# 0xPARC/plonkathon

Measured on NVIDIA H100. Metric: plonk_proofs_per_s_2^20_gates, higher is better.
Workload: dtype u256 (BN254 Fr/Fq integers, 8x32-bit Montgomery limbs)

## Files before the change

plonkathon_b200/csrc/capi.cu:

```cuda
#include "../../include/plonk_b200.h"

#include <cstring>

#include "common.cuh"
#include "comm.cuh"
#include "msm_bucket.cuh"
#include "prover.cuh"
#include "pairing.cuh"
#include "transcript.cuh"

namespace pb200 {
void ntt_run(Context* ctx, const Fr* in, Fr* out, int log_n, bool inverse, uint64_t n_in, const Fr* in_scale,
             const Fr* out_scale);
void launch_powers(Context* ctx, Fr* out, uint64_t n, const Fr& base, const Fr& scale);
Fr fr_from_u64(uint64_t x);
void ntt_run_strided(Context* ctx, const Fr* in, Fr* out, int log_n, bool inverse, uint64_t n_in,
                     const Fr* in_scale, const Fr* out_scale, uint64_t in_mul, uint64_t in_add);
void ntt_sharded(Context* ctx, const Fr* const* in, Fr* const* out, int count, int log_n, bool inverse);
void fr_to_mont(Context* ctx, const Fr* in, Fr* out, uint64_t n);
void fr_from_mont(Context* ctx, const Fr* in, Fr* out, uint64_t n);
void fr_vec_op(Context* ctx, int op, const Fr* a, const Fr* b, const Fr& scalar_canonical, Fr* out, uint64_t n,
               uint64_t shift);
void barycentric_eval(Context* ctx, const Fr* d_vals, int log_n, const Fr& x_mont, Fr* h_out);
float bench_modmul(Context* ctx, int field, uint64_t threads, uint32_t iters);
struct Srs;
Srs* srs_create(Context* ctx, const uint8_t* h_points, uint64_t n, int precompute);
void srs_destroy(Srs* s);
Srs* srs_generate(Context* ctx, const Fr& tau_canonical, uint64_t n, int precompute);
Srs* srs_generate_lagrange(Context* ctx, const Fr& tau_canonical, uint64_t n, int precompute);
void srs_export(Context* ctx, Srs* srs, uint8_t* h_points, uint64_t first, uint64_t count);
void srs_msm(Context* ctx, Srs* srs, const Fr* d_scalars, uint64_t m, bool scalars_mont, uint8_t* out_xy, int* is_identity);
uint64_t srs_size(Srs* s);
uint32_t msm_default_window(uint64_t n, bool fixed_base);
void msm_run(Context* ctx, const G1Affine* points, uint64_t n, const Fr* scalars, bool scalars_mont, uint32_t c,
             bool fixed_base, uint64_t point_stride, uint8_t* out_xy, int* is_identity);
void affine_to_mont(Context* ctx, const G1Affine* in, G1Affine* out, uint64_t n);
Prover* prover_create(Context* ctx, Srs* srs, int log_n, const uint8_t* const* h_pk, int n_custom,
                      const uint8_t* h_exps, const uint8_t* const* h_custom, bool sharded, int exp_width);
void prover_destroy(Prover* p);
void prover_prove(Prover* P, const uint8_t* hA, const uint8_t* hB, const uint8_t* hC, const uint8_t* h_public,
                  uint64_t n_public, uint8_t* out, bool wires_on_device);
void prover_round1(Prover* P, const uint8_t* hA, const uint8_t* hB, const uint8_t* hC, const uint8_t* h_public,
                   uint64_t n_public, bool wires_on_device);
void prover_round2(Prover* P, const Fr* ch);
void prover_round3(Prover* P, const Fr& alpha_c, const Fr& cofactor_c);
void prover_round4(Prover* P, const Fr& zeta_c);
void prover_round5(Prover* P, const Fr& v_c);
void prover_serialize(const Prover* P, uint8_t* out);
size_t copy_step(const Prover* P, int step, uint8_t* out);
void prover_set_zk(Prover* P, unsigned block, bool enable, const uint8_t* h_blinders);
void prover_set_lookup(Prover* P, const uint8_t* h_qk, const uint8_t* h_qtag, const uint8_t* const* h_tab,
                       uint64_t rows);
void prover_round_lookup(Prover* P, const Fr& eta_c);
void prover_set_shuffle(Prover* P, const uint8_t* h_qin, const uint8_t* h_qout);
void g1_combine_partials_host(const G1XYZZ* parts, uint32_t count, uint8_t* out_xy, int* is_identity);
void host_join_bucket_shards(const SR* all, uint32_t world, uint32_t sets, uint32_t nloc, G1XYZZ* out);
void host_join_bucket_shards_strided(const SR* all, uint32_t world, uint32_t sets, G1XYZZ* out);
void prover_check(Prover* P, const uint8_t* hA, const uint8_t* hB, const uint8_t* hC, const uint8_t* h_public,
                  uint64_t n_public, uint32_t limit, uint64_t* h_counts, uint32_t* h_lists, bool wires_on_device);
void permutation_run(Context* ctx, const int64_t* h_ids, int log_n, uint8_t* h_S);
Srs* srs_create_ptau(Context* ctx, const uint8_t* h_g1, uint64_t count, const uint8_t* h_tau_g2, int precompute);
Srs* srs_create_ptau_lagrange(Context* ctx, const uint8_t* h_block, uint64_t n, Srs* monomial, int precompute);
void ptau_stages(double* out_ms, int count);

const Bn254Pairing& pairing_engine() {
  static const Bn254Pairing engine;
  return engine;
}
}

using namespace pb200;

static thread_local std::string g_err;

#define PB_API_BEGIN try {
#define PB_API_END                        \
  return 0;                               \
  }                                       \
  catch (const std::exception& e) {       \
    g_err = e.what();                     \
    return 1;                             \
  }                                       \
  catch (...) {                           \
    g_err = "unknown error";              \
    return 1;                             \
  }
// ... 67 lines not shown
                  const uint8_t* y, uint8_t* out) {
  PB_API_BEGIN PB_ON_CTX(reinterpret_cast<Prover*>(p)->ctx);
  Prover* P = reinterpret_cast<Prover*>(p);
  require_kind(P, kind, "round2", STEP_2);
  Fr ch[PROOF_CHALLENGES] = {};
  ch[CH_BETA] = load_fr_canonical(beta);
  ch[CH_GAMMA] = load_fr_canonical(gamma);
  if (kind != BLOCK_PLAIN) {
    const bool sh = kind & BLOCK_SHUFFLE;
    ch[sh ? CH_THETA : CH_DELTA] = load_fr_canonical(x);
    ch[sh ? CH_KAPPA : CH_EPSILON] = load_fr_canonical(y);
  }
  prover_round2(P, ch);
  copy_step(P, STEP_2, out);
  PB_API_END
}
static int round4(pb200_prover* p, unsigned kind, const uint8_t* zeta, uint8_t* out) {
  PB_API_BEGIN PB_ON_CTX(reinterpret_cast<Prover*>(p)->ctx);
  Prover* P = reinterpret_cast<Prover*>(p);
  require_kind(P, kind, "round4", STEP_4);
  prover_round4(P, load_fr_canonical(zeta));
  copy_step(P, STEP_4, out);
  PB_API_END
}
static int set_zk(pb200_prover* p, unsigned block, int enable, const uint8_t* h_blinders) {
  PB_API_BEGIN PB_ON_CTX(reinterpret_cast<Prover*>(p)->ctx);
  prover_set_zk(reinterpret_cast<Prover*>(p), block, enable != 0, h_blinders);
  PB_API_END
}

extern "C" {

const char* pb200_last_error(void) { return g_err.c_str(); }
const char* pb200_version(void) { return "plonk_b200 0.1 (sm_90a)"; }

int pb200_ctx_create(int device, void* cuda_stream, pb200_ctx** out) {
  PB_API_BEGIN
  int count = 0;
  cudaError_t e = cudaGetDeviceCount(&count);
  PB_CHECK(e == cudaSuccess && count > 0, "no CUDA device: libplonk_b200 has no CPU fallback");
  PB_CHECK(device >= 0 && device < count, "bad device ordinal");
  PB_CUDA(cudaSetDevice(device));
  auto ctx = std::make_unique<Context>();
  ctx->device = device;
  cudaDeviceProp prop;
  PB_CUDA(cudaGetDeviceProperties(&prop, device));
  ctx->sm_count = prop.multiProcessorCount;
  if (cuda_stream) {
    ctx->stream = reinterpret_cast<cudaStream_t>(cuda_stream);
  } else {
    PB_CUDA(cudaStreamCreateWithFlags(&ctx->stream, cudaStreamNonBlocking));
    ctx->own_stream = true;
  }
  *out = reinterpret_cast<pb200_ctx*>(ctx.release());
  PB_API_END
}

void pb200_ctx_destroy(pb200_ctx* ctx) {
  if (!ctx) return;
  cudaSetDevice(C(ctx)->device);
  cudaStreamSynchronize(C(ctx)->stream);
  delete C(ctx);
}

int pb200_ctx_sync(pb200_ctx* ctx) {
  PB_API_BEGIN PB_ON_CTX(C(ctx));
  PB_CUDA(cudaStreamSynchronize(C(ctx)->stream));
  PB_API_END
}

uint64_t pb200_ctx_launches(pb200_ctx* ctx) { return C(ctx)->launches; }

int pb200_ctx_timing(pb200_ctx* ctx, int enable) {
  PB_API_BEGIN PB_ON_CTX(C(ctx));
  Context* c = C(ctx);
  PB_CUDA(cudaStreamSynchronize(c->stream));
  for (auto& v : c->timed) {
    for (auto& pr : v) { cudaEventDestroy(pr.first); cudaEventDestroy(pr.second); }
    v.clear();
  }
  c->timing = enable != 0;
  PB_API_END
}
int pb200_ctx_timing_read(pb200_ctx* ctx, int category, double* total_ms, uint64_t* count) {
  PB_API_BEGIN PB_ON_CTX(C(ctx));
  Context* c = C(ctx);
  PB_CHECK(category >= 0 && category < 4, "bad timing category");
  PB_CUDA(cudaStreamSynchronize(c->stream));
  double t = 0;
  for (auto& pr : c->timed[category]) {
    float ms = 0;
    PB_CUDA(cudaEventElapsedTime(&ms, pr.first, pr.second));
    t += ms;
  }
  *total_ms = t;
  *count = c->timed[category].size();
  PB_API_END
}
void* pb200_ctx_stream(pb200_ctx* ctx) { return (void*)C(ctx)->stream; }

int pb200_fr_to_mont(pb200_ctx* ctx, const void* d_in, void* d_out, uint64_t n) {
  PB_API_BEGIN PB_ON_CTX(C(ctx));
  fr_to_mont(C(ctx), (const Fr*)d_in, (Fr*)d_out, n);
  PB_API_END
}
int pb200_fr_from_mont(pb200_ctx* ctx, const void* d_in, void* d_out, uint64_t n) {
// ... 582 lines not shown
```

plonkathon_b200/csrc/common.cuh:

```cuda
#pragma once
#include <cuda_runtime.h>
#include <stdint.h>
#include <stdio.h>
#include <map>
#include <memory>
#include <stdexcept>
#include <string>
#include <vector>

#include "curve.cuh"
#include "field.cuh"
#include "modinv.cuh"

namespace pb200 {

struct Error : std::runtime_error {
  using std::runtime_error::runtime_error;
};

#define PB_CUDA(expr)                                                                          \
  do {                                                                                         \
    cudaError_t e__ = (expr);                                                                  \
    if (e__ != cudaSuccess) {                                                                  \
      char b__[512];                                                                           \
      snprintf(b__, sizeof b__, "%s failed: %s (%s:%d)", #expr, cudaGetErrorString(e__),       \
               __FILE__, __LINE__);                                                            \
      throw pb200::Error(b__);                                                                 \
    }                                                                                          \
  } while (0)

#define PB_CHECK(cond, msg)                                                                    \
  do {                                                                                         \
    if (!(cond)) {                                                                             \
      char b__[512];                                                                           \
      snprintf(b__, sizeof b__, "%s (%s:%d)", msg, __FILE__, __LINE__);                        \
      throw pb200::Error(b__);                                                                 \
    }                                                                                          \
  } while (0)

struct DevBuf {
  void* p = nullptr;
  size_t bytes = 0;
  DevBuf() {}
  explicit DevBuf(size_t n) { alloc(n); }
  DevBuf(const DevBuf&) = delete;
  DevBuf& operator=(const DevBuf&) = delete;
  DevBuf(DevBuf&& o) noexcept : p(o.p), bytes(o.bytes) { o.p = nullptr; o.bytes = 0; }
  DevBuf& operator=(DevBuf&& o) noexcept {
    if (this != &o) { release(); p = o.p; bytes = o.bytes; o.p = nullptr; o.bytes = 0; }
    return *this;
  }
  ~DevBuf() { release(); }
  void alloc(size_t n) {
    release();
    if (n) PB_CUDA(cudaMalloc(&p, n));
    bytes = n;
  }
  void ensure(size_t n) { if (n > bytes) alloc(n); }
  void release() { if (p) cudaFree(p); p = nullptr; bytes = 0; }
  template <class T> T* as() const { return reinterpret_cast<T*>(p); }
};

struct NttPlan;
struct Srs;
struct Comm;
struct ShardTables;

struct Context {
  int device = 0;
  cudaStream_t stream = nullptr;
  bool own_stream = false;
  cudaStream_t aux_stream = nullptr;
  cudaEvent_t aux_ev[4] = {nullptr, nullptr, nullptr, nullptr};
  cudaStream_t copy_stream = nullptr;
  cudaEvent_t copy_done[4] = {nullptr, nullptr, nullptr, nullptr};
  int sm_count = 132;
  std::map<int, std::unique_ptr<NttPlan>> plans;
  DevBuf scratch[10];
  DevBuf msm_aff[6];
  Comm* comm = nullptr;
  DevBuf gather;
  std::map<int, std::unique_ptr<ShardTables>> shard_tables;
  uint64_t launches = 0;
  bool timing = false;
  std::vector<std::pair<cudaEvent_t, cudaEvent_t>> timed[4];
  void time_begin(int cat) {
    if (!timing) return;
    cudaEvent_t a, b;
    cudaEventCreate(&a);
    cudaEventCreate(&b);
    cudaEventRecord(a, stream);
    timed[cat].push_back({a, b});
  }
  void time_end(int cat) {
    if (!timing) return;
    cudaEventRecord(timed[cat].back().second, stream);
  }
  Context();
  ~Context();
};

NttPlan* get_plan(Context* ctx, int log_n, bool inverse);

}
```

plonkathon_b200/csrc/msm.cu:

```cuda
#include <algorithm>
#include <cstring>

#include "common.cuh"
#include "comm.cuh"
#include "msm_bucket.cuh"
#include "msm_digits.cuh"
#include "msm_sort.cuh"

namespace pb200 {

__device__ __forceinline__ G1Affine ld_affine(const G1Affine* p) {
  const uint4* q = reinterpret_cast<const uint4*>(p);
  uint4 a = __ldg(q), b = __ldg(q + 1), c = __ldg(q + 2), d = __ldg(q + 3);
  G1Affine r;
  r.x.v[0] = a.x; r.x.v[1] = a.y; r.x.v[2] = a.z; r.x.v[3] = a.w;
  r.x.v[4] = b.x; r.x.v[5] = b.y; r.x.v[6] = b.z; r.x.v[7] = b.w;
  r.y.v[0] = c.x; r.y.v[1] = c.y; r.y.v[2] = c.z; r.y.v[3] = c.w;
  r.y.v[4] = d.x; r.y.v[5] = d.y; r.y.v[6] = d.z; r.y.v[7] = d.w;
  return r;
}

__device__ __forceinline__ uint32_t block_exclusive_scan(uint32_t v, uint32_t* sh, uint32_t* total) {
  const uint32_t lane = threadIdx.x & 31, wid = threadIdx.x >> 5, nw = blockDim.x >> 5;
  uint32_t x = v;
  for (int d = 1; d < 32; d <<= 1) {
    uint32_t y = __shfl_up_sync(0xffffffffu, x, d);
    if ((int)lane >= d) x += y;
  }
  if (lane == 31) sh[wid] = x;
  __syncthreads();
  if (wid == 0) {
    uint32_t w = lane < nw ? sh[lane] : 0;
    for (int d = 1; d < 32; d <<= 1) {
      uint32_t y = __shfl_up_sync(0xffffffffu, w, d);
      if ((int)lane >= d) w += y;
    }
    if (lane < nw) sh[lane] = w;
  }
  __syncthreads();
  uint32_t base = wid ? sh[wid - 1] : 0;
  *total = sh[nw - 1];
  __syncthreads();
  return base + x - v;
}

__global__ void __launch_bounds__(PB_SORT_BIN_THREADS) k_msm_bin_count(SortArgs a) {
  __shared__ uint32_t sh_cnt[PB_SORT_MAX_BINS];
  const uint32_t t = threadIdx.x, nt = blockDim.x;
  sort_zero(sh_cnt, a.nbins, t, nt);
  __syncthreads();
  bin_hist(a, blockIdx.x, blockIdx.y, t, nt, sh_cnt);
  __syncthreads();
  bin_flush(a, t, nt, sh_cnt);
}

__global__ void __launch_bounds__(PB_SORT_BIN_THREADS) k_msm_bin_scatter(SortArgs a) {
  __shared__ uint32_t sh_cnt[PB_SORT_MAX_BINS], sh_loc[PB_SORT_MAX_BINS], sh_base[PB_SORT_MAX_BINS], sh_scan[32];
  extern __shared__ SortEntry stage[];
  const uint32_t t = threadIdx.x, nt = blockDim.x;
  sort_zero(sh_cnt, a.nbins, t, nt);
  __syncthreads();
  bin_hist(a, blockIdx.x, blockIdx.y, t, nt, sh_cnt);
  __syncthreads();
  uint32_t total;
  const uint32_t run = block_exclusive_scan(scan_part_sum(sh_cnt, a.nbins, t, nt), sh_scan, &total);
  bin_reserve(a, t, nt, run, sh_cnt, sh_loc, sh_base);
  __syncthreads();
  bin_stage(a, blockIdx.x, blockIdx.y, t, nt, sh_cnt, sh_loc, stage);
  __syncthreads();
  bin_copy_out(a, t, nt, total, sh_loc, sh_base, stage);
}

__global__ void __launch_bounds__(PB_SORT_CHUNK_THREADS) k_msm_chunk_count(SortArgs a) {
  __shared__ uint32_t sh_cnt[PB_SORT_MAX_BIN_KEYS];
  const uint32_t t = threadIdx.x, nt = blockDim.x;
  SortChunk ch;
  for (uint32_t c = blockIdx.x; chunk_locate(a, c, ch); c += gridDim.x) {
    sort_zero(sh_cnt, ch.nkeys, t, nt);
    __syncthreads();
    chunk_hist(a, ch, t, nt, sh_cnt);
    __syncthreads();
    chunk_flush(a, ch, t, nt, sh_cnt);
    __syncthreads();
  }
}

__global__ void __launch_bounds__(PB_SORT_CHUNK_THREADS) k_msm_chunk_place(SortArgs a) {
  __shared__ uint32_t sh_cnt[PB_SORT_MAX_BIN_KEYS], sh_loc[PB_SORT_MAX_BIN_KEYS], sh_base[PB_SORT_MAX_BIN_KEYS],
      sh_scan[32];
  extern __shared__ uint32_t stage_vals[];
  const uint32_t t = threadIdx.x, nt = blockDim.x;
  SortChunk ch;
  for (uint32_t c = blockIdx.x; chunk_locate(a, c, ch); c += gridDim.x) {
    sort_zero(sh_cnt, ch.nkeys, t, nt);
    __syncthreads();
    chunk_hist(a, ch, t, nt, sh_cnt);
    __syncthreads();
    uint32_t total;
    const uint32_t run = block_exclusive_scan(scan_part_sum(sh_cnt, ch.nkeys, t, nt), sh_scan, &total);
    chunk_reserve(a, ch, t, nt, run, sh_cnt, sh_loc, sh_base);
    __syncthreads();
    chunk_stage(a, ch, t, nt, sh_cnt, sh_loc, stage_vals);
    __syncthreads();
    chunk_copy_out(a, ch, t, nt, sh_loc, sh_base, stage_vals);
    __syncthreads();
  }
}

#define PB_SCAN_TILE 2048
// ... 82 lines not shown

__device__ __forceinline__ uint32_t upper_bound_u32(const uint32_t* a, uint32_t n, uint32_t key) {
  uint32_t lo = 0, hi = n;
  while (lo < hi) {
    uint32_t mid = (lo + hi) >> 1;
    if (__ldg(a + mid) > key) hi = mid; else lo = mid + 1;
  }
  return lo;
}

__global__ void __launch_bounds__(128, 4) k_msm_seg_accumulate(const G1Affine* points, const uint32_t* offsets,
                                                            const uint32_t* sorted, uint32_t nb, uint32_t L,
                                                            G1XYZZ* buckets, G1XYZZ* slots, uint32_t* slot_bucket,
                                                            uint32_t* own_slot) {
  const uint32_t t = blockIdx.x * blockDim.x + threadIdx.x;
  const uint32_t M = offsets[nb];
  const uint64_t s64 = (uint64_t)t * L;
  if (s64 >= M) return;
  const uint32_t s = (uint32_t)s64;
  const uint32_t e = (uint32_t)min((uint64_t)M, s64 + L);
  uint32_t b = upper_bound_u32(offsets, nb + 1, s) - 1;
  uint32_t bstart = offsets[b], bend = offsets[b + 1];
  bool first = true;
  G1XYZZ acc = G1XYZZ::identity();
  for (uint32_t pos = s; pos <= e; pos++) {
    if (pos == bend || pos == e) {
      if (bstart >= s && bend <= e) {
        buckets[b] = acc;
      } else {
        uint32_t slot = first ? 2 * t : 2 * t + 1;
        slots[slot] = acc;
        slot_bucket[slot] = b;
        if (bstart >= s) own_slot[t] = slot;
      }
      if (pos == e) break;
      first = false;
      acc = G1XYZZ::identity();
      b++;
      while (offsets[b + 1] <= pos) b++;
      bstart = offsets[b];
      bend = offsets[b + 1];
    }
    uint32_t v = __ldg(sorted + pos);
    G1Affine p = ld_affine(points + (v & 0x7fffffffu));
    if (v >> 31) p.y = fp_neg(p.y);
    g1_add_mixed_uniform(acc, p);
  }
}

struct HeavyItem { uint32_t bucket, own_slot, t0, t1, piece_base, pieces; };
struct HeavyPiece { uint32_t item, index; };
#define PB_STITCH_PIECE 1024

__global__ void __launch_bounds__(128) k_msm_stitch(const uint32_t* offsets, uint32_t nb, uint32_t L,
                                                    uint32_t n_segments, const G1XYZZ* slots,
                                                    const uint32_t* slot_bucket, const uint32_t* own_slot,
                                                    G1XYZZ* buckets, HeavyItem* heavy, uint32_t* heavy_count,
                                                    HeavyPiece* pieces, uint32_t small_limit) {
  const uint32_t t = blockIdx.x * blockDim.x + threadIdx.x;
  if (t >= n_segments) return;
  const uint32_t os = own_slot[t];
  if (os == PB_MSM_EMPTY) return;
  const uint32_t b = slot_bucket[os];
  const uint32_t t1 = (offsets[b + 1] - 1) / L;
  if (t1 - t > small_limit) {
    uint32_t h = atomicAdd(heavy_count, 1u);
    HeavyItem it; it.bucket = b; it.own_slot = os; it.t0 = t; it.t1 = t1; it.piece_base = 0; it.pieces = 0;
    if (t1 - t > PB_STITCH_PIECE) {
      it.pieces = (t1 - t + PB_STITCH_PIECE - 1) / PB_STITCH_PIECE;
      it.piece_base = atomicAdd(heavy_count + 1, it.pieces);
      for (uint32_t p = 0; p < it.pieces; p++) { HeavyPiece hp; hp.item = h; hp.index = p; pieces[it.piece_base + p] = hp; }
    }
    heavy[h] = it;
    return;
  }
  G1XYZZ acc = slots[os];
  for (uint32_t k = t + 1; k <= t1; k++) {
    G1XYZZ piece = slots[2 * k];
    g1_add(acc, piece);
  }
  buckets[b] = acc;
}

__device__ __forceinline__ void block_sum_xyzz(G1XYZZ* sh, const G1XYZZ& mine) {
  sh[threadIdx.x] = mine;
  __syncthreads();
  for (uint32_t d = blockDim.x >> 1; d > 0; d >>= 1) {
    if (threadIdx.x < d) {
      G1XYZZ a = sh[threadIdx.x], c = sh[threadIdx.x + d];
      g1_add(a, c);
      sh[threadIdx.x] = a;
    }
    __syncthreads();
  }
}

__global__ void __launch_bounds__(128) k_msm_stitch_pieces(const G1XYZZ* slots, const HeavyItem* heavy,
                                                           const uint32_t* heavy_count, const HeavyPiece* pieces,
                                                           G1XYZZ* partial) {
  __shared__ G1XYZZ sh[128];
  const uint32_t count = heavy_count[1];
  for (uint32_t p = blockIdx.x; p < count; p += gridDim.x) {
    const HeavyPiece hp = pieces[p];
    const HeavyItem it = heavy[hp.item];
    const uint32_t lo = it.t0 + 1 + hp.index * PB_STITCH_PIECE;
    const uint32_t hi = min(lo + PB_STITCH_PIECE - 1, it.t1);
    G1XYZZ acc = G1XYZZ::identity();
    for (uint32_t k = lo + threadIdx.x; k <= hi; k += blockDim.x) {
      G1XYZZ piece = slots[2 * k];
      g1_add(acc, piece);
    }
    block_sum_xyzz(sh, acc);
    if (threadIdx.x == 0) partial[p] = sh[0];
    __syncthreads();
  }
}

__global__ void __launch_bounds__(128) k_msm_stitch_heavy(const G1XYZZ* slots, const HeavyItem* heavy,
                                                          const uint32_t* heavy_count, const G1XYZZ* partial,
                                                          G1XYZZ* buckets) {
  __shared__ G1XYZZ sh[128];
  const uint32_t count = *heavy_count;
  for (uint32_t h = blockIdx.x; h < count; h += gridDim.x) {
    HeavyItem it = heavy[h];
    G1XYZZ acc = G1XYZZ::identity();
    if (threadIdx.x == 0) acc = slots[it.own_slot];
    if (it.pieces) {
      for (uint32_t p = threadIdx.x; p < it.pieces; p += blockDim.x) {
        G1XYZZ piece = partial[it.piece_base + p];
        g1_add(acc, piece);
      }
    } else {
      for (uint32_t k = it.t0 + 1 + threadIdx.x; k <= it.t1; k += blockDim.x) {
        G1XYZZ piece = slots[2 * k];
        g1_add(acc, piece);
      }
    }
    block_sum_xyzz(sh, acc);
    if (threadIdx.x == 0) buckets[it.bucket] = sh[0];
    __syncthreads();
  }
}

__global__ void __launch_bounds__(128) k_reduce_level0(ReduceArgs a) {
  reduce_level0_thread(a, (uint64_t)blockIdx.x * blockDim.x + threadIdx.x);
}
__global__ void __launch_bounds__(PB_REDUCE_THREADS) k_reduce_block(BlockLevelArgs a) {
  __shared__ G1XYZZ sh[PB_REDUCE_THREADS];
  const uint32_t t = threadIdx.x, chunk = blockIdx.x, set = blockIdx.y;
  G1XYZZ s, x;
  blk_local(a, set, chunk, t, s, x);
  sh[t] = s;
  __syncthreads();
#pragma unroll 1
  for (uint32_t d = 1; d < PB_REDUCE_THREADS; d <<= 1) {
    const G1XYZZ v = blk_scan_step(sh, t, d);
    __syncthreads();
    sh[t] = v;
    __syncthreads();
  }
  const G1XYZZ suf = sh[t];
  const G1XYZZ y = blk_weight(a, t, x, suf);
  __syncthreads();
  sh[t] = y;
  __syncthreads();
#pragma unroll 1
  for (uint32_t d = PB_REDUCE_THREADS / 2; d > 0; d >>= 1) {
    blk_tree_step(sh, t, d);
    __syncthreads();
  }
  if (t == 0) {
// ... 21 lines not shown
  p.y = fp_from_mont(p.y);
  out[i] = p;
}

__global__ void __launch_bounds__(128) k_window_step(const G1Affine* in, G1XYZZ* out, uint64_t n, uint32_t c) {
  uint64_t i = (uint64_t)blockIdx.x * blockDim.x + threadIdx.x;
  if (i >= n) return;
  G1Affine p = in[i];
  G1XYZZ a;
  g1_double_affine(a, p);
  for (uint32_t k = 1; k < c; k++) g1_double(a);
  out[i] = a;
}

void affine_to_mont(Context* ctx, const G1Affine* in, G1Affine* out, uint64_t n) {
  k_affine_to_mont<<<(unsigned)((n + 127) / 128), 128, 0, ctx->stream>>>(in, out, n);
  ctx->launches++;
  PB_CUDA(cudaGetLastError());
}

__global__ void __launch_bounds__(128) k_batch_to_affine(const G1XYZZ* in, G1Affine* out, uint64_t n) {
  const int CH = 16;
  uint64_t t = (uint64_t)blockIdx.x * blockDim.x + threadIdx.x;
  uint64_t i0 = t * CH;
  if (i0 >= n) return;
  int cnt = (int)min((uint64_t)CH, n - i0);
  Fq pref[CH];
  Fq run = Fq::one();
  for (int k = 0; k < cnt; k++) {
    pref[k] = run;
    run = fp_mul(run, in[i0 + k].ZZZ);
  }
  Fq inv = fp_inv_gcd(run);
  for (int k = cnt - 1; k >= 0; k--) {
    G1XYZZ a = in[i0 + k];
    Fq A = fp_mul(inv, pref[k]);
    inv = fp_mul(inv, a.ZZZ);
    Fq izz = fp_sqr(fp_mul(a.ZZ, A));
    G1Affine p;
    p.x = fp_mul(a.X, izz);
    p.y = fp_mul(a.Y, A);
    out[i0 + k] = p;
  }
}

struct Srs {
  uint64_t n = 0;
  DevBuf base;
  uint32_t c = 0, W = 0;
  DevBuf expanded;
};

static uint32_t windows_for(uint32_t c) { return (256 + c - 1) / c; }

uint32_t msm_default_window(uint64_t n, bool fixed_base) {
  int lg = 0;
  while (((uint64_t)1 << lg) < n) lg++;
  int c = fixed_base ? lg : lg - 4;
  int lo = 4, hi = fixed_base ? 21 : 16;
  if (const char* e = getenv(fixed_base ? "PB200_MSM_C_FIXED" : "PB200_MSM_C")) { c = atoi(e); }
  if (c < lo) c = lo;
  if (c > hi) c = hi;
  return (uint32_t)c;
}

static G1XYZZ host_mul_small(const G1XYZZ& p, uint32_t k) {
  G1XYZZ r = G1XYZZ::identity();
  for (int i = 31; i >= 0; i--) {
    g1_double(r);
    if ((k >> i) & 1) g1_add(r, p);
  }
  return r;
}

static void host_horner_to_affine(const std::vector<G1XYZZ>& ws, uint32_t c, uint8_t* out_xy, int* is_identity) {
  G1XYZZ r = G1XYZZ::identity();
  for (int w = (int)ws.size() - 1; w >= 0; w--) {
    if (w != (int)ws.size() - 1)
      for (uint32_t k = 0; k < c; k++) g1_double(r);
    g1_add(r, ws[w]);
  }
  G1Affine a;
  bool inf = g1_to_affine(r, a);
  *is_identity = inf ? 1 : 0;
  Fq x = fp_from_mont(a.x), y = fp_from_mont(a.y);
  memcpy(out_xy, x.v, 32);
  memcpy(out_xy + 32, y.v, 32);
}

static uint32_t env_u32(const char* name, uint32_t dflt) {
  const char* e = getenv(name);
  return e ? (uint32_t)atoi(e) : dflt;
}

static uint32_t pick_B(Context* ctx, uint64_t slots, uint32_t r) {
  static const uint32_t forced = env_u32("PB200_MSM_B", 0);
  const uint32_t cap = r == 0 ? 64 : PB_AFF_BMAX;
  if (forced) return std::min<uint32_t>(std::max<uint32_t>(r == 0 ? forced : 2 * forced, 2), cap);
  const uint64_t full = (uint64_t)ctx->sm_count * 256;
  for (uint32_t B = cap; B > 16; B >>= 1)
    if (slots / aff_round_span(B, r) >= 2 * full) return B;
  return 16;
}

void host_join_bucket_shards_strided(const SR* all, uint32_t world, uint32_t sets, G1XYZZ* out) {
  uint32_t log_g = 0;
// ... 75 lines not shown
  g.nb = g.sets * g.nloc;
  PB_CHECK((fixed_base ? (uint64_t)g.W * point_stride : n) < (1ull << 31), "MSM too large for 31-bit point ids");
  ScalarBatch sb;
  for (uint32_t k = 0; k < 4; k++) sb.p[k] = k < batch ? scalars[k] : nullptr;

  static const bool use_xyzz = [] { const char* e = getenv("PB200_MSM_ACC"); return !(e && !strcmp(e, "affine")); }();
  const uint32_t pad = use_xyzz ? 0 : 1;
  DevBuf& sorted = ctx->scratch[2];
  DevBuf& counts = ctx->scratch[3];
  DevBuf& offsets = ctx->scratch[4];
  DevBuf& lvl_a = ctx->scratch[6];
  DevBuf& lvl_b = ctx->scratch[7];
  const uint64_t entries = n * g.W * batch;
  const uint64_t positions = entries + (pad ? g.nb : 0);
  PB_CHECK(positions < (1ull << 30), "MSM too large (n * windows * batch must stay below 2^30)");
  sorted.ensure(positions * 4);
  counts.ensure((size_t)g.nb * 4 + 16);
  offsets.ensure((size_t)(g.nb + 1) * 4);
  uint32_t* max_cnt = counts.as<uint32_t>() + g.nb;
  const uint32_t n_tiles = (g.nb + PB_SCAN_TILE - 1) / PB_SCAN_TILE;
  PB_CHECK(n_tiles <= 8192, "too many buckets for the scan");
  ctx->msm_aff[1].ensure((size_t)8192 * 4);
  uint32_t* tile_sums = ctx->msm_aff[1].as<uint32_t>();

  const uint32_t lb = sort_default_lb(g.nb);
  PB_CHECK((1u << lb) <= PB_SORT_MAX_BIN_KEYS, "too many buckets for the sort");
  DevBuf& binned = ctx->scratch[8];
  DevBuf& bin_tab = ctx->scratch[9];
  binned.ensure(entries * sizeof(SortEntry));
  bin_tab.ensure((size_t)3 * (PB_SORT_MAX_BINS + 1) * 4);
  SortArgs sa;
  sa.sb = sb;
  sa.n = n;
  sa.from_mont = scalars_mont ? 1 : 0;
  sa.g = g;
  sa.lb = lb;
  sa.nbins = ((g.nb - 1) >> lb) + 1;
  sa.T = PB_SORT_CHUNK;
  uint32_t* bin_cnt = bin_tab.as<uint32_t>();
  uint32_t* bin_off = bin_cnt + PB_SORT_MAX_BINS + 1;
  sa.bin_cnt = bin_cnt;
  sa.bin_off = bin_off;
  sa.binned = binned.as<SortEntry>();
  sa.chunk_first = bin_off + PB_SORT_MAX_BINS + 1;
  sa.counts = counts.as<uint32_t>();
  sa.offsets = offsets.as<uint32_t>();
  sa.sorted = sorted.as<uint32_t>();
  sa.spb = PB_SORT_BIN_STAGE / g.W;
  const dim3 bin_grid((unsigned)((n + sa.spb - 1) / sa.spb), batch);
  const uint64_t chunk_bound = entries / PB_SORT_CHUNK + sa.nbins;
  const uint32_t count_grid = (uint32_t)std::min<uint64_t>((uint64_t)ctx->sm_count * 4, chunk_bound);
  const uint32_t place_grid = (uint32_t)std::min<uint64_t>((uint64_t)ctx->sm_count * 2, chunk_bound);
  const size_t bin_stage_bytes = PB_SORT_BIN_STAGE * sizeof(SortEntry), chunk_stage_bytes = PB_SORT_CHUNK * 4;
  PB_CUDA(cudaFuncSetAttribute(k_msm_bin_scatter, cudaFuncAttributeMaxDynamicSharedMemorySize, (int)bin_stage_bytes));
  PB_CUDA(cudaFuncSetAttribute(k_msm_chunk_place, cudaFuncAttributeMaxDynamicSharedMemorySize, (int)chunk_stage_bytes));

  cudaStream_t st = ctx->stream;
  ctx->time_begin(2);
  PB_CUDA(cudaMemsetAsync(counts.p, 0, (size_t)g.nb * 4 + 16, st));
  PB_CUDA(cudaMemsetAsync(bin_cnt, 0, (size_t)sa.nbins * 4, st));
  if (pad) PB_CUDA(cudaMemsetAsync(sorted.p, 0xff, positions * 4, st));
  k_msm_bin_count<<<bin_grid, PB_SORT_BIN_THREADS, 0, st>>>(sa);
  k_scan_tile_sums<<<1, 256, 0, st>>>(bin_cnt, sa.nbins, 0, tile_sums, nullptr);
  k_scan_tiles<<<1, 256, 0, st>>>(tile_sums, 1, bin_off + sa.nbins);
  k_scan_apply<<<1, 256, 0, st>>>(bin_cnt, sa.nbins, 0, tile_sums, bin_off);
  k_msm_bin_scatter<<<bin_grid, PB_SORT_BIN_THREADS, bin_stage_bytes, st>>>(sa);
  k_msm_chunk_map<<<1, 256, 0, st>>>(sa);
  k_msm_chunk_count<<<count_grid, PB_SORT_CHUNK_THREADS, 0, st>>>(sa);
  k_scan_tile_sums<<<n_tiles, 256, 0, st>>>(counts.as<uint32_t>(), g.nb, pad, tile_sums, max_cnt);
  k_scan_tiles<<<1, 256, 0, st>>>(tile_sums, n_tiles, offsets.as<uint32_t>() + g.nb);
  k_scan_apply<<<n_tiles, 256, 0, st>>>(counts.as<uint32_t>(), g.nb, pad, tile_sums, offsets.as<uint32_t>());
  k_msm_chunk_place<<<place_grid, PB_SORT_CHUNK_THREADS, chunk_stage_bytes, st>>>(sa);
  ctx->time_end(2);
  ctx->launches += 11;

  ReduceArgs ra;
  ra.pts = nullptr; ra.off = offsets.as<uint32_t>(); ra.cnt = counts.as<uint32_t>(); ra.xb = nullptr;
  if (!use_xyzz) {
    const uint64_t s_bound = positions / 2;
    DevBuf& pts = ctx->msm_aff[0];
    pts.ensure(s_bound * sizeof(G1Affine));
    AffAcc a;
    a.table = points;
    a.sorted = sorted.as<uint32_t>();
    a.pts = pts.as<G1Affine>();
    a.off = offsets.as<uint32_t>();
    a.cnt = counts.as<uint32_t>();
    a.max_cnt = max_cnt;
    a.nbl = g.nb;
    uint64_t cap = fixed_base ? n * g.W : n;
    uint32_t max_rounds = 1;
    while (max_rounds < 32 && (1ull << max_rounds) < cap) max_rounds++;
    ctx->time_begin(0);
    for (uint32_t r = 0; r < std::min<uint32_t>(max_rounds, PB_AFF_GRID_ROUNDS); r++) {
      a.r = r;
      a.B = pick_B(ctx, s_bound, r);
      const uint64_t threads = aff_round_threads(s_bound, a.B, r);
      if (r == 0) k_aff_round0<<<(unsigned)((threads + 127) / 128), 128, 0, st>>>(a);
      else k_aff_round<<<(unsigned)((threads + 127) / 128), 128, 0, st>>>(a);
      ctx->launches++;
    }
    if (max_rounds > PB_AFF_GRID_ROUNDS) {
      a.B = 32;
      k_aff_tail<<<1, 256, 0, st>>>(a, s_bound);
      ctx->launches++;
    }
    ctx->time_end(0);
    ra.pts = pts.as<G1Affine>();
  } else {
    DevBuf& buckets = ctx->scratch[5];
    DevBuf& seg = ctx->scratch[1];
    buckets.ensure((size_t)g.nb * sizeof(G1XYZZ));
    static const uint32_t seg_env = env_u32("PB200_MSM_SEG", 0);
    uint32_t L = 32;
    if (seg_env) {
      L = seg_env;
    } else {
      const uint64_t expected = entries / (g.half / g.nloc);
      while (L > 4 && expected / L < (uint64_t)ctx->sm_count * 512) L >>= 1;
      while (L < 32 && (entries / L) * (2 * sizeof(G1XYZZ) + 12 + sizeof(HeavyItem)) > (1ull << 30)) L <<= 1;
    }
    PB_CHECK(L >= 1 && L <= 4096, "bad PB200_MSM_SEG");
    const uint32_t n_seg = (uint32_t)((entries + L - 1) / L);
    const uint32_t max_pieces = 2 * (n_seg / PB_STITCH_PIECE) + 16;
    seg.ensure((size_t)n_seg * 2 * sizeof(G1XYZZ) + (size_t)n_seg * 3 * 4 + (size_t)n_seg * sizeof(HeavyItem) + 16 +
               (size_t)max_pieces * (sizeof(HeavyPiece) + sizeof(G1XYZZ)));
    G1XYZZ* slots = seg.as<G1XYZZ>();
    G1XYZZ* piece_partial = slots + (size_t)n_seg * 2;
    uint32_t* slot_bucket = reinterpret_cast<uint32_t*>(piece_partial + max_pieces);
    uint32_t* own_slot = slot_bucket + (size_t)n_seg * 2;
    uint32_t* heavy_count = own_slot + n_seg;
    HeavyItem* heavy = reinterpret_cast<HeavyItem*>(heavy_count + 4);
    HeavyPiece* pieces = reinterpret_cast<HeavyPiece*>(heavy + n_seg);
    PB_CUDA(cudaMemsetAsync(buckets.p, 0, (size_t)g.nb * sizeof(G1XYZZ), st));
    PB_CUDA(cudaMemsetAsync(own_slot, 0xff, (size_t)n_seg * 4, st));
    PB_CUDA(cudaMemsetAsync(heavy_count, 0, 16, st));
    ctx->time_begin(0);
    k_msm_seg_accumulate<<<(n_seg + 127) / 128, 128, 0, st>>>(points, offsets.as<uint32_t>(), sorted.as<uint32_t>(),
                                                             g.nb, L, buckets.as<G1XYZZ>(), slots, slot_bucket, own_slot);
    ctx->time_end(0);
    k_msm_stitch<<<(n_seg + 127) / 128, 128, 0, st>>>(offsets.as<uint32_t>(), g.nb, L, n_seg, slots, slot_bucket,
                                                     own_slot, buckets.as<G1XYZZ>(), heavy, heavy_count, pieces, 16);
    k_msm_stitch_pieces<<<std::min<uint32_t>(max_pieces, 592), 128, 0, st>>>(slots, heavy, heavy_count, pieces, piece_partial);
    k_msm_stitch_heavy<<<296, 128, 0, st>>>(slots, heavy, heavy_count, piece_partial, buckets.as<G1XYZZ>());
    ctx->launches += 4;
    ra.xb = buckets.as<G1XYZZ>();
  }

  static const uint32_t g0_env = env_u32("PB200_MSM_G", 0);
  uint32_t log_g0 = 4;
  if (g0_env) {
    log_g0 = 1;
    while ((2u << log_g0) <= g0_env && log_g0 < 10) log_g0++;
  } else {
    while (log_g0 > 2 && (g.nb >> log_g0) < (uint32_t)ctx->sm_count * 256) log_g0--;
  }
  ctx->time_begin(3);
  ra.sets = g.sets;
  ra.m = g.nloc;
  ra.g = 1u << log_g0;
  {
    const uint64_t groups = (uint64_t)g.sets * reduce_groups(ra.m, ra.g);
    lvl_a.ensure(groups * sizeof(SR));
    lvl_b.ensure((groups / 16 + g.sets) * sizeof(SR));
    ra.out = lvl_a.as<SR>();
    k_reduce_level0<<<(unsigned)((groups + 127) / 128), 128, 0, st>>>(ra);
    ctx->launches++;
  }
  uint32_t m = reduce_groups(ra.m, ra.g), log_G = log_g0;
  SR* cur = lvl_a.as<SR>();
  SR* nxt = lvl_b.as<SR>();
  const uint32_t m_stop = comm ? 1 : 8;
  while (m > m_stop) {
    BlockLevelArgs ba;
    ba.in = cur; ba.out = nxt; ba.sets = g.sets; ba.m = m; ba.log_G = log_G;
    k_reduce_block<<<dim3(reduce_chunks(m), g.sets), PB_REDUCE_THREADS, 0, st>>>(ba);
    ctx->launches++;
    m = reduce_chunks(m);
    log_G += 9;
    std::swap(cur, nxt);
  }
  ctx->time_end(3);
  PB_CUDA(cudaGetLastError());
  std::vector<G1XYZZ> ws(g.sets);
  if (comm) {
    const uint32_t world = (uint32_t)comm_world(comm);
    DevBuf& gath = ctx->msm_aff[2];
    const size_t per_rank = (size_t)g.sets * m;
    gath.ensure((size_t)world * per_rank * sizeof(SR));
    SR* all = gath.as<SR>();
    PB_CUDA(cudaMemcpyAsync(all + (size_t)comm_rank(comm) * per_rank, cur, per_rank * sizeof(SR), cudaMemcpyDeviceToDevice, st));
    comm_allgather_inplace(comm, all, per_rank * sizeof(SR), st);
    std::vector<SR> raw((size_t)world * per_rank), fin((size_t)world * g.sets);
    PB_CUDA(cudaMemcpyAsync(raw.data(), all, raw.size() * sizeof(SR), cudaMemcpyDeviceToHost, st));
    PB_CUDA(cudaStreamSynchronize(st));
    for (uint32_t rho = 0; rho < world; rho++)
      for (uint32_t s = 0; s < g.sets; s++)
        fin[(size_t)rho * g.sets + s] = reduce_fold_final(raw.data() + (size_t)rho * per_rank + (size_t)s * m, m, log_G);
    if (g.own_log) host_join_bucket_shards_strided(fin.data(), world, g.sets, ws.data());
    else host_join_bucket_shards(fin.data(), world, g.sets, g.nloc, ws.data());
  } else {
    std::vector<SR> raw((size_t)g.sets * m), fin(g.sets);
    PB_CUDA(cudaMemcpyAsync(raw.data(), cur, raw.size() * sizeof(SR), cudaMemcpyDeviceToHost, st));
    PB_CUDA(cudaStreamSynchronize(st));
    for (uint32_t s = 0; s < g.sets; s++) fin[s] = reduce_fold_final(raw.data() + (size_t)s * m, m, log_G);
    for (uint32_t s = 0; s < g.sets; s++) {
      ws[s] = fin[s].R;
      if (g.lo) {
        G1XYZZ m_lo = host_mul_small(fin[s].S, g.lo);
        g1_add(ws[s], m_lo);
      }
    }
  }
  if (raw_out) {
    if (fixed_base) {
      for (uint32_t k = 0; k < batch; k++) raw_out[k] = ws[k];
    } else {
      G1XYZZ r = G1XYZZ::identity();
      for (int w = (int)g.W - 1; w >= 0; w--) {
        if (w != (int)g.W - 1) for (uint32_t k = 0; k < c; k++) g1_double(r);
        g1_add(r, ws[w]);
      }
      raw_out[0] = r;
    }
  } else if (fixed_base) {
    for (uint32_t k = 0; k < batch; k++) {
      std::vector<G1XYZZ> one(1, ws[k]);
      host_horner_to_affine(one, c, out_xy + 64 * k, is_identity + k);
    }
  } else {
    host_horner_to_affine(ws, c, out_xy, is_identity);
  }
}

void msm_run(Context* ctx, const G1Affine* points, uint64_t n, const Fr* scalars, bool scalars_mont, uint32_t c,
// ... 191 lines not shown
```

plonkathon_b200/csrc/ntt.cu:

```cuda
#include "common.cuh"
#include "comm.cuh"
#include "ntt_shard.cuh"

namespace pb200 {

Fr fr_from_u64(uint64_t x) {
  Fr a = Fr::zero();
  a.v[0] = (uint32_t)x;
  a.v[1] = (uint32_t)(x >> 32);
  return fp_to_mont(a);
}

Fr fr_root_of_unity(int log_n) {
  uint32_t e[8];
  for (int i = 0; i < 8; i++) e[i] = FrParams::p(i);
  e[0] -= 1;
  for (int s = 0; s < log_n; s++) {
    for (int i = 0; i < 8; i++) e[i] = (e[i] >> 1) | (i < 7 ? (e[i + 1] << 31) : 0);
  }
  return fp_pow(fr_from_u64(5), e);
}

__global__ void k_gen_interpass(Fr* out, uint64_t rows, uint64_t cols, Fr w, Fr scale) {
  const int CH = 64;
// ... 354 lines not shown
      ctx->launches++;
      q.twg = ps.twg.as<Fr>();
    } else {
      q.twg = nullptr;
      q.b_fastest_load = 1;
      ps.log_cc = std::min(std::max(0, kTileLog - lb[i]), lb[0]);
      uint64_t CC = (uint64_t)1 << ps.log_cc;
      if (npass == 2) {
        batch = N1;
        q.t_lo_count = 1;
        q.r_hi = CC * N2; q.r_lo = 0; q.r_cs = N2; q.r_bs = 1;
        q.w_hi = CC; q.w_lo = 0; q.w_cs = 1; q.w_bs = N1;
      } else {
        batch = N1;
        q.t_lo_count = (uint32_t)N2;
        q.r_hi = CC * N2 * N3; q.r_lo = N3; q.r_cs = N2 * N3; q.r_bs = 1;
        q.w_hi = CC; q.w_lo = N1; q.w_cs = 1; q.w_bs = N1 * N2;
      }
    }
    (void)batch;
    q.log_cc = ps.log_cc;
    q.log_n = log_n;
    q.fold = 1;
    ps.tiles = N >> (lb[i] + ps.log_cc);
    size_t smem = pass_smem_bytes(ps.log_b, ps.log_cc);
    PB_CHECK(smem <= 227 * 1024, "NTT tile does not fit shared memory");
  }
  PB_CUDA(cudaGetLastError());
  return plan;
}

NttPlan* get_plan(Context* ctx, int log_n, bool inverse) {
  int key = log_n * 2 + (inverse ? 1 : 0);
  auto it = ctx->plans.find(key);
  if (it != ctx->plans.end()) return it->second.get();
  if (ctx->plans.empty())
    PB_CUDA(cudaFuncSetAttribute(k_ntt_pass, cudaFuncAttributeMaxDynamicSharedMemorySize, 227 * 1024));
  auto plan = build_plan(ctx, log_n, inverse);
  NttPlan* raw = plan.get();
  ctx->plans[key] = std::move(plan);
  return raw;
}

Context::Context() {}

Context::~Context() {
  plans.clear();
  shard_tables.clear();
  if (comm) comm_destroy(comm);
  for (auto& e : copy_done) if (e) cudaEventDestroy(e);
  for (auto& e : aux_ev) if (e) cudaEventDestroy(e);
  if (aux_stream) cudaStreamDestroy(aux_stream);
  if (copy_stream) cudaStreamDestroy(copy_stream);
  if (own_stream && stream) cudaStreamDestroy(stream);
}

void ntt_run_strided(Context* ctx, const Fr* in, Fr* out, int log_n, bool inverse, uint64_t n_in,
                     const Fr* in_scale, const Fr* out_scale, uint64_t in_mul, uint64_t in_add);

void ntt_run(Context* ctx, const Fr* in, Fr* out, int log_n, bool inverse, uint64_t n_in,
             const Fr* in_scale, const Fr* out_scale) {
  ntt_run_strided(ctx, in, out, log_n, inverse, n_in, in_scale, out_scale, 1, 0);
}

void ntt_run_on(Context* ctx, cudaStream_t stream, Fr* tmp, const Fr* in, Fr* out, int log_n, bool inverse,
                uint64_t n_in, const Fr* in_scale, const Fr* out_scale, uint64_t in_mul, uint64_t in_add);
void ntt_run_fold(Context* ctx, cudaStream_t stream, Fr* tmp, const Fr* in, Fr* out, int log_n, bool inverse,
                  uint64_t n_in, const Fr* in_scale, const Fr* out_scale, uint64_t in_mul, uint64_t in_add, uint32_t fold);

void ntt_run_strided(Context* ctx, const Fr* in, Fr* out, int log_n, bool inverse, uint64_t n_in,
                     const Fr* in_scale, const Fr* out_scale, uint64_t in_mul, uint64_t in_add) {
  ntt_run_on(ctx, ctx->stream, nullptr, in, out, log_n, inverse, n_in, in_scale, out_scale, in_mul, in_add);
}

void ntt_run_on(Context* ctx, cudaStream_t stream, Fr* tmp, const Fr* in, Fr* out, int log_n, bool inverse,
                uint64_t n_in, const Fr* in_scale, const Fr* out_scale, uint64_t in_mul, uint64_t in_add) {
  ntt_run_fold(ctx, stream, tmp, in, out, log_n, inverse, n_in, in_scale, out_scale, in_mul, in_add, 1);
}

void ntt_run_fold(Context* ctx, cudaStream_t stream, Fr* tmp, const Fr* in, Fr* out, int log_n, bool inverse,
                  uint64_t n_in, const Fr* in_scale, const Fr* out_scale, uint64_t in_mul, uint64_t in_add, uint32_t fold) {
  NttPlan* plan = get_plan(ctx, log_n, inverse);
  const uint64_t N = (uint64_t)1 << log_n;
  int np = (int)plan->passes.size();
  const bool main_stream = stream == ctx->stream;
  if (np > 1 && !tmp) {
    PB_CHECK(main_stream, "a side-stream transform needs its own pass buffer");
    ctx->scratch[0].ensure((size_t)N * 32);
    tmp = ctx->scratch[0].as<Fr>();
  }
  for (int i = 0; i < np; i++) {
    NttPass& ps = plan->passes[i];
    PassParams q = ps.prm;
    q.in = (i == 0) ? in : tmp;
    q.out = (i == np - 1) ? out : tmp;
    q.n_in = (i == 0) ? n_in : N;
    q.in_mul = (i == 0) ? in_mul : 1;
    q.in_add = (i == 0) ? in_add : 0;
    q.in_scale = (i == 0) ? in_scale : nullptr;
    q.out_scale = (i == np - 1) ? out_scale : nullptr;
    q.fold = (i == 0) ? fold : 1;
    size_t smem = pass_smem_bytes(ps.log_b, ps.log_cc);
    if (main_stream) ctx->time_begin(1);
    k_ntt_pass<<<(unsigned)ps.tiles, PB_NTT_THREADS, smem, stream>>>(q);
    if (main_stream) ctx->time_end(1);
    ctx->launches++;
// ... 108 lines not shown
```

Before: 23.87.

## Run MSM sort, stitch and reduce phases on a high-priority stream

Adds a high-priority stream and a join event to the context and moves the MSM sort, bucket stitch and tree-reduce kernels onto it, joining back to the main stream at each dependency. The intent is that latency-critical, low-occupancy MSM phases get scheduled ahead of work queued on other streams such as aux or copy work. Kernel shared-memory attributes are now set once at context creation instead of on every MSM call, and several MSM kernels get a minimum-blocks-per-SM of 4 in their launch bounds. The joins run strictly in sequence, so little real overlap is added, and one shared join event reused across many joins could be fragile if it is ever used concurrently.

```diff
diff --git a/plonkathon_b200/csrc/capi.cu b/plonkathon_b200/csrc/capi.cu
--- a/plonkathon_b200/csrc/capi.cu
+++ b/plonkathon_b200/csrc/capi.cu
@@ -32,6 +32,7 @@
 void srs_msm(Context* ctx, Srs* srs, const Fr* d_scalars, uint64_t m, bool scalars_mont, uint8_t* out_xy, int* is_identity);
 uint64_t srs_size(Srs* s);
 uint32_t msm_default_window(uint64_t n, bool fixed_base);
+void msm_init_device();
 void msm_run(Context* ctx, const G1Affine* points, uint64_t n, const Fr* scalars, bool scalars_mont, uint32_t c,
              bool fixed_base, uint64_t point_stride, uint8_t* out_xy, int* is_identity);
 void affine_to_mont(Context* ctx, const G1Affine* in, G1Affine* out, uint64_t n);
@@ -205,6 +206,11 @@
     PB_CUDA(cudaStreamCreateWithFlags(&ctx->stream, cudaStreamNonBlocking));
     ctx->own_stream = true;
   }
+  int prio_least = 0, prio_greatest = 0;
+  PB_CUDA(cudaDeviceGetStreamPriorityRange(&prio_least, &prio_greatest));
+  PB_CUDA(cudaStreamCreateWithPriority(&ctx->prio_stream, cudaStreamNonBlocking, prio_greatest));
+  PB_CUDA(cudaEventCreateWithFlags(&ctx->join_ev, cudaEventDisableTiming));
+  msm_init_device();
   *out = reinterpret_cast<pb200_ctx*>(ctx.release());
   PB_API_END
 }
diff --git a/plonkathon_b200/csrc/common.cuh b/plonkathon_b200/csrc/common.cuh
--- a/plonkathon_b200/csrc/common.cuh
+++ b/plonkathon_b200/csrc/common.cuh
@@ -74,6 +74,8 @@
   cudaEvent_t aux_ev[4] = {nullptr, nullptr, nullptr, nullptr};
   cudaStream_t copy_stream = nullptr;
   cudaEvent_t copy_done[4] = {nullptr, nullptr, nullptr, nullptr};
+  cudaStream_t prio_stream = nullptr;
+  cudaEvent_t join_ev = nullptr;
   int sm_count = 132;
   std::map<int, std::unique_ptr<NttPlan>> plans;
   DevBuf scratch[10];
@@ -84,17 +86,17 @@
   uint64_t launches = 0;
   bool timing = false;
   std::vector<std::pair<cudaEvent_t, cudaEvent_t>> timed[4];
-  void time_begin(int cat) {
+  void time_begin(int cat, cudaStream_t on = nullptr) {
     if (!timing) return;
     cudaEvent_t a, b;
     cudaEventCreate(&a);
     cudaEventCreate(&b);
-    cudaEventRecord(a, stream);
+    cudaEventRecord(a, on ? on : stream);
     timed[cat].push_back({a, b});
   }
-  void time_end(int cat) {
+  void time_end(int cat, cudaStream_t on = nullptr) {
     if (!timing) return;
-    cudaEventRecord(timed[cat].back().second, stream);
+    cudaEventRecord(timed[cat].back().second, on ? on : stream);
   }
   Context();
   ~Context();
@@ -102,4 +104,9 @@
 
 NttPlan* get_plan(Context* ctx, int log_n, bool inverse);
 
+inline void stream_join(Context* ctx, cudaStream_t waiter, cudaStream_t producer) {
+  PB_CUDA(cudaEventRecord(ctx->join_ev, producer));
+  PB_CUDA(cudaStreamWaitEvent(waiter, ctx->join_ev, 0));
 }
+
+}
diff --git a/plonkathon_b200/csrc/msm.cu b/plonkathon_b200/csrc/msm.cu
--- a/plonkathon_b200/csrc/msm.cu
+++ b/plonkathon_b200/csrc/msm.cu
@@ -44,7 +44,7 @@
   return base + x - v;
 }
 
-__global__ void __launch_bounds__(PB_SORT_BIN_THREADS) k_msm_bin_count(SortArgs a) {
+__global__ void __launch_bounds__(PB_SORT_BIN_THREADS, 4) k_msm_bin_count(SortArgs a) {
   __shared__ uint32_t sh_cnt[PB_SORT_MAX_BINS];
   const uint32_t t = threadIdx.x, nt = blockDim.x;
   sort_zero(sh_cnt, a.nbins, t, nt);
@@ -54,7 +54,7 @@
   bin_flush(a, t, nt, sh_cnt);
 }
 
-__global__ void __launch_bounds__(PB_SORT_BIN_THREADS) k_msm_bin_scatter(SortArgs a) {
+__global__ void __launch_bounds__(PB_SORT_BIN_THREADS, 4) k_msm_bin_scatter(SortArgs a) {
   __shared__ uint32_t sh_cnt[PB_SORT_MAX_BINS], sh_loc[PB_SORT_MAX_BINS], sh_base[PB_SORT_MAX_BINS], sh_scan[32];
   extern __shared__ SortEntry stage[];
   const uint32_t t = threadIdx.x, nt = blockDim.x;
@@ -243,7 +243,7 @@
 struct HeavyPiece { uint32_t item, index; };
 #define PB_STITCH_PIECE 1024
 
-__global__ void __launch_bounds__(128) k_msm_stitch(const uint32_t* offsets, uint32_t nb, uint32_t L,
+__global__ void __launch_bounds__(128, 4) k_msm_stitch(const uint32_t* offsets, uint32_t nb, uint32_t L,
                                                     uint32_t n_segments, const G1XYZZ* slots,
                                                     const uint32_t* slot_bucket, const uint32_t* own_slot,
                                                     G1XYZZ* buckets, HeavyItem* heavy, uint32_t* heavy_count,
@@ -286,7 +286,7 @@
   }
 }
 
-__global__ void __launch_bounds__(128) k_msm_stitch_pieces(const G1XYZZ* slots, const HeavyItem* heavy,
+__global__ void __launch_bounds__(128, 4) k_msm_stitch_pieces(const G1XYZZ* slots, const HeavyItem* heavy,
                                                            const uint32_t* heavy_count, const HeavyPiece* pieces,
                                                            G1XYZZ* partial) {
   __shared__ G1XYZZ sh[128];
@@ -307,7 +307,7 @@
   }
 }
 
-__global__ void __launch_bounds__(128) k_msm_stitch_heavy(const G1XYZZ* slots, const HeavyItem* heavy,
+__global__ void __launch_bounds__(128, 4) k_msm_stitch_heavy(const G1XYZZ* slots, const HeavyItem* heavy,
                                                           const uint32_t* heavy_count, const G1XYZZ* partial,
                                                           G1XYZZ* buckets) {
   __shared__ G1XYZZ sh[128];
@@ -435,6 +435,12 @@
 };
 
 static uint32_t windows_for(uint32_t c) { return (256 + c - 1) / c; }
+
+void msm_init_device() {
+  PB_CUDA(cudaFuncSetAttribute(k_msm_bin_scatter, cudaFuncAttributeMaxDynamicSharedMemorySize,
+                               (int)(PB_SORT_BIN_STAGE * sizeof(SortEntry))));
+  PB_CUDA(cudaFuncSetAttribute(k_msm_chunk_place, cudaFuncAttributeMaxDynamicSharedMemorySize, (int)(PB_SORT_CHUNK * 4)));
+}
 
 uint32_t msm_default_window(uint64_t n, bool fixed_base) {
   int lg = 0;
@@ -616,26 +622,25 @@
   const uint32_t count_grid = (uint32_t)std::min<uint64_t>((uint64_t)ctx->sm_count * 4, chunk_bound);
   const uint32_t place_grid = (uint32_t)std::min<uint64_t>((uint64_t)ctx->sm_count * 2, chunk_bound);
   const size_t bin_stage_bytes = PB_SORT_BIN_STAGE * sizeof(SortEntry), chunk_stage_bytes = PB_SORT_CHUNK * 4;
-  PB_CUDA(cudaFuncSetAttribute(k_msm_bin_scatter, cudaFuncAttributeMaxDynamicSharedMemorySize, (int)bin_stage_bytes));
-  PB_CUDA(cudaFuncSetAttribute(k_msm_chunk_place, cudaFuncAttributeMaxDynamicSharedMemorySize, (int)chunk_stage_bytes));
-
-  cudaStream_t st = ctx->stream;
-  ctx->time_begin(2);
-  PB_CUDA(cudaMemsetAsync(counts.p, 0, (size_t)g.nb * 4 + 16, st));
-  PB_CUDA(cudaMemsetAsync(bin_cnt, 0, (size_t)sa.nbins * 4, st));
-  if (pad) PB_CUDA(cudaMemsetAsync(sorted.p, 0xff, positions * 4, st));
-  k_msm_bin_count<<<bin_grid, PB_SORT_BIN_THREADS, 0, st>>>(sa);
-  k_scan_tile_sums<<<1, 256, 0, st>>>(bin_cnt, sa.nbins, 0, tile_sums, nullptr);
-  k_scan_tiles<<<1, 256, 0, st>>>(tile_sums, 1, bin_off + sa.nbins);
-  k_scan_apply<<<1, 256, 0, st>>>(bin_cnt, sa.nbins, 0, tile_sums, bin_off);
-  k_msm_bin_scatter<<<bin_grid, PB_SORT_BIN_THREADS, bin_stage_bytes, st>>>(sa);
-  k_msm_chunk_map<<<1, 256, 0, st>>>(sa);
-  k_msm_chunk_count<<<count_grid, PB_SORT_CHUNK_THREADS, 0, st>>>(sa);
-  k_scan_tile_sums<<<n_tiles, 256, 0, st>>>(counts.as<uint32_t>(), g.nb, pad, tile_sums, max_cnt);
-  k_scan_tiles<<<1, 256, 0, st>>>(tile_sums, n_tiles, offsets.as<uint32_t>() + g.nb);
-  k_scan_apply<<<n_tiles, 256, 0, st>>>(counts.as<uint32_t>(), g.nb, pad, tile_sums, offsets.as<uint32_t>());
-  k_msm_chunk_place<<<place_grid, PB_SORT_CHUNK_THREADS, chunk_stage_bytes, st>>>(sa);
-  ctx->time_end(2);
+
+  cudaStream_t st = ctx->stream, ps = ctx->prio_stream;
+  stream_join(ctx, ps, st);
+  ctx->time_begin(2, ps);
+  PB_CUDA(cudaMemsetAsync(counts.p, 0, (size_t)g.nb * 4 + 16, ps));
+  PB_CUDA(cudaMemsetAsync(bin_cnt, 0, (size_t)sa.nbins * 4, ps));
+  if (pad) PB_CUDA(cudaMemsetAsync(sorted.p, 0xff, positions * 4, ps));
+  k_msm_bin_count<<<bin_grid, PB_SORT_BIN_THREADS, 0, ps>>>(sa);
+  k_scan_tile_sums<<<1, 256, 0, ps>>>(bin_cnt, sa.nbins, 0, tile_sums, nullptr);
+  k_scan_tiles<<<1, 256, 0, ps>>>(tile_sums, 1, bin_off + sa.nbins);
+  k_scan_apply<<<1, 256, 0, ps>>>(bin_cnt, sa.nbins, 0, tile_sums, bin_off);
+  k_msm_bin_scatter<<<bin_grid, PB_SORT_BIN_THREADS, bin_stage_bytes, ps>>>(sa);
+  k_msm_chunk_map<<<1, 256, 0, ps>>>(sa);
+  k_msm_chunk_count<<<count_grid, PB_SORT_CHUNK_THREADS, 0, ps>>>(sa);
+  k_scan_tile_sums<<<n_tiles, 256, 0, ps>>>(counts.as<uint32_t>(), g.nb, pad, tile_sums, max_cnt);
+  k_scan_tiles<<<1, 256, 0, ps>>>(tile_sums, n_tiles, offsets.as<uint32_t>() + g.nb);
+  k_scan_apply<<<n_tiles, 256, 0, ps>>>(counts.as<uint32_t>(), g.nb, pad, tile_sums, offsets.as<uint32_t>());
+  k_msm_chunk_place<<<place_grid, PB_SORT_CHUNK_THREADS, chunk_stage_bytes, ps>>>(sa);
+  ctx->time_end(2, ps);
   ctx->launches += 11;
 
   ReduceArgs ra;
@@ -655,6 +660,7 @@
     uint64_t cap = fixed_base ? n * g.W : n;
     uint32_t max_rounds = 1;
     while (max_rounds < 32 && (1ull << max_rounds) < cap) max_rounds++;
+    stream_join(ctx, st, ps);
     ctx->time_begin(0);
     for (uint32_t r = 0; r < std::min<uint32_t>(max_rounds, PB_AFF_GRID_ROUNDS); r++) {
       a.r = r;
@@ -696,20 +702,23 @@
     uint32_t* heavy_count = own_slot + n_seg;
     HeavyItem* heavy = reinterpret_cast<HeavyItem*>(heavy_count + 4);
     HeavyPiece* pieces = reinterpret_cast<HeavyPiece*>(heavy + n_seg);
-    PB_CUDA(cudaMemsetAsync(buckets.p, 0, (size_t)g.nb * sizeof(G1XYZZ), st));
-    PB_CUDA(cudaMemsetAsync(own_slot, 0xff, (size_t)n_seg * 4, st));
-    PB_CUDA(cudaMemsetAsync(heavy_count, 0, 16, st));
+    PB_CUDA(cudaMemsetAsync(buckets.p, 0, (size_t)g.nb * sizeof(G1XYZZ), ps));
+    PB_CUDA(cudaMemsetAsync(own_slot, 0xff, (size_t)n_seg * 4, ps));
+    PB_CUDA(cudaMemsetAsync(heavy_count, 0, 16, ps));
+    stream_join(ctx, st, ps);
     ctx->time_begin(0);
     k_msm_seg_accumulate<<<(n_seg + 127) / 128, 128, 0, st>>>(points, offsets.as<uint32_t>(), sorted.as<uint32_t>(),
                                                              g.nb, L, buckets.as<G1XYZZ>(), slots, slot_bucket, own_slot);
     ctx->time_end(0);
-    k_msm_stitch<<<(n_seg + 127) / 128, 128, 0, st>>>(offsets.as<uint32_t>(), g.nb, L, n_seg, slots, slot_bucket,
+    stream_join(ctx, ps, st);
+    k_msm_stitch<<<(n_seg + 127) / 128, 128, 0, ps>>>(offsets.as<uint32_t>(), g.nb, L, n_seg, slots, slot_bucket,
                                                      own_slot, buckets.as<G1XYZZ>(), heavy, heavy_count, pieces, 16);
-    k_msm_stitch_pieces<<<std::min<uint32_t>(max_pieces, 592), 128, 0, st>>>(slots, heavy, heavy_count, pieces, piece_partial);
-    k_msm_stitch_heavy<<<296, 128, 0, st>>>(slots, heavy, heavy_count, piece_partial, buckets.as<G1XYZZ>());
+    k_msm_stitch_pieces<<<std::min<uint32_t>(max_pieces, 592), 128, 0, ps>>>(slots, heavy, heavy_count, pieces, piece_partial);
+    k_msm_stitch_heavy<<<296, 128, 0, ps>>>(slots, heavy, heavy_count, piece_partial, buckets.as<G1XYZZ>());
     ctx->launches += 4;
     ra.xb = buckets.as<G1XYZZ>();
   }
+  stream_join(ctx, st, ps);
 
   static const uint32_t g0_env = env_u32("PB200_MSM_G", 0);
   uint32_t log_g0 = 4;
@@ -731,6 +740,7 @@
     k_reduce_level0<<<(unsigned)((groups + 127) / 128), 128, 0, st>>>(ra);
     ctx->launches++;
   }
+  stream_join(ctx, ps, st);
   uint32_t m = reduce_groups(ra.m, ra.g), log_G = log_g0;
   SR* cur = lvl_a.as<SR>();
   SR* nxt = lvl_b.as<SR>();
@@ -738,13 +748,14 @@
   while (m > m_stop) {
     BlockLevelArgs ba;
     ba.in = cur; ba.out = nxt; ba.sets = g.sets; ba.m = m; ba.log_G = log_G;
-    k_reduce_block<<<dim3(reduce_chunks(m), g.sets), PB_REDUCE_THREADS, 0, st>>>(ba);
+    k_reduce_block<<<dim3(reduce_chunks(m), g.sets), PB_REDUCE_THREADS, 0, ps>>>(ba);
     ctx->launches++;
     m = reduce_chunks(m);
     log_G += 9;
     std::swap(cur, nxt);
   }
-  ctx->time_end(3);
+  ctx->time_end(3, ps);
+  stream_join(ctx, st, ps);
   PB_CUDA(cudaGetLastError());
   std::vector<G1XYZZ> ws(g.sets);
   if (comm) {
diff --git a/plonkathon_b200/csrc/ntt.cu b/plonkathon_b200/csrc/ntt.cu
--- a/plonkathon_b200/csrc/ntt.cu
+++ b/plonkathon_b200/csrc/ntt.cu
@@ -430,6 +430,8 @@
   for (auto& e : aux_ev) if (e) cudaEventDestroy(e);
   if (aux_stream) cudaStreamDestroy(aux_stream);
   if (copy_stream) cudaStreamDestroy(copy_stream);
+  if (join_ev) cudaEventDestroy(join_ev);
+  if (prio_stream) cudaStreamDestroy(prio_stream);
   if (own_stream && stream) cudaStreamDestroy(stream);
 }
 
```

Result: faster. 25.46 (median of 6 runs) (+6.7%).
